# DJjjjhao/FIRA-ICSE

Measured on AMD Instinct MI355X. Metric: training commits/sec (FIRA default config), higher is better.
Workload: dtype f32; 1 GPU; BASELINE configs[1]: FIRA training step (fwd+bwd+Adam, dropout 0.1/0.2), batch 32 commits/GPU, fp32, 650-node graphs (mean nnz 1066/graph), vocab 24650; global_batch=32, parallelism=dp1

## Files before the change

fira_icse_amd/csrc/engine.h:

```cpp
#pragma once
#include "common.h"
#include <string>
#include <vector>

namespace fira {

int gemm_f32(hipStream_t s, int tA, int tB, int M, int N, int K, const float* A, int lda, const float* B, int ldb,
             float* C, int ldc, const float* bias, int flags, int splitk);
int gemm_f32_ex(hipStream_t s, int tA, int tB, int M, int N, int K, const float* A, int lda, const float* B, int ldb,
                float* C, int ldc, const float* bias, int flags, int splitk, float* colsum,
                const int32_t* c_rows = nullptr, const float* relu_mask = nullptr);
int gemm_bf16_ex(hipStream_t s, int tA, int tB, int M, int N, int K, const float* A, int lda, const float* B, int ldb,
                 float* C, int ldc, const float* bias, int flags, int splitk, float* colsum,
                 const int32_t* c_rows = nullptr, const float* relu_mask = nullptr);
struct ShadowEntry { int64_t offset; int rows, cols, pitch_t; int64_t offset_t; };
constexpr int SHADOW_MAX = 64;
struct ShadowTable {
    int n = 0;
    int64_t wbt_elems = 0;
    int tile_start[SHADOW_MAX + 1] = {0};
    ShadowEntry e[SHADOW_MAX];
};
int weight_shadows(hipStream_t s, const ShadowTable& tab, const float* P, uint16_t* Wb, uint16_t* WbT);
int gemm_bf16_wb_ex(hipStream_t s, int M, int N, int K, const float* A, int lda, const uint16_t* Bb, int ldb, float* C,
                    int ldc, const float* bias, int flags, int splitk, const int32_t* c_rows = nullptr,
                    const float* relu_mask = nullptr);
bool gemm_bf16_takes(int M, int N, int K);
struct GroupProblem {
    const float* A;
    const float* B;
    float* C;
    float* colsum;
    int M, N, K, lda, ldb, ldc, tiles_m, tiles_n, splitk, k_chunk;
};
constexpr int GROUP_MAX = 40;
struct GroupTable {
    int n = 0, chunk = 0;
    int wg_start[GROUP_MAX + 1] = {0};
    GroupProblem p[GROUP_MAX];
    void cost(double& flop, double& bytes) const {
        flop = bytes = 0;
        for (int i = 0; i < n; ++i) {
            const double M = p[i].M, N = p[i].N, K = p[i].K;
            flop += 2.0 * M * N * K;
            bytes += 4.0 * (M * K + N * K + M * N);
        }
    }
};
int gemm_group_plan(GroupProblem& q, int max_split);
int gemm_group_launch(hipStream_t s, const GroupTable& t);
int gemm_bf16_group_plan(GroupProblem& q, int max_split);
int gemm_bf16_group_launch(hipStream_t s, GroupTable& t);
struct PanelProblem {
    const float *A, *B;
    float *C, *colsum;
    float* part;
    int M, N, K, lda, ldb, ldc;
    int tiles_m, tiles_n, slabs, k_slab;
};
constexpr int PANEL_MAX = 48;
struct PanelTable {
    int n = 0;
    int wg_start[PANEL_MAX + 1] = {0};
    PanelProblem p[PANEL_MAX];
};
bool gemm_wgrad_panel_takes(int M, int N, int K, const float* A, int lda, const float* B, int ldb, int ldc);
int gemm_wgrad_panel_launch(hipStream_t s, int np, PanelTable& t, float* scratch, size_t scratch_floats);
struct WgradQueue {
    GroupTable tiled;
    PanelTable panels;
    float* scratch = nullptr;
    size_t scratch_floats = 0;
    int dtype = 0;
    void reset(int dtype_, float* scratch_, size_t floats) {
        tiled.n = 0; panels.n = 0;
        dtype = dtype_; scratch = scratch_; scratch_floats = scratch_ ? floats : 0;
    }
    bool full() const { return tiled.n == GROUP_MAX || panels.n == PANEL_MAX; }
    int panel_pending() const { return panels.n; }
    int add_tiled(int M, int N, int K, const float* A, int lda, const float* B, int ldb, float* C, int ldc, float* colsum,
                  int max_split = 0) {
        if (M <= 0 || N <= 0 || K <= 0) return 0;
        FIRA_REQUIRE(tiled.n < GROUP_MAX, "wgrad queue: tiled group full (fork and flush first)");
        GroupProblem& q = tiled.p[tiled.n];
        q.A = A; q.B = B; q.C = C; q.colsum = colsum;
        q.M = M; q.N = N; q.K = K; q.lda = lda; q.ldb = ldb; q.ldc = ldc;
        q.tiles_m = cdiv(M, 64); q.tiles_n = cdiv(N, 64);
        if (int rc = dtype == 1 ? gemm_bf16_group_plan(q, max_split) : gemm_group_plan(q, max_split)) return rc;
        tiled.wg_start[tiled.n + 1] = tiled.wg_start[tiled.n] + q.tiles_m * q.tiles_n * q.splitk;
        ++tiled.n;
        return 0;
    }
    int add_panel(int M, int N, int K, const float* A, int lda, const float* B, int ldb, float* C, int ldc, float* colsum) {
        FIRA_REQUIRE(panels.n < PANEL_MAX, "wgrad queue: panel table full (fork and flush first)");
        PanelProblem& q = panels.p[panels.n++];
        q.A = A; q.B = B; q.C = C; q.colsum = colsum;
        q.M = M; q.N = N; q.K = K; q.lda = lda; q.ldb = ldb; q.ldc = ldc;
        q.tiles_m = cdiv(M, 256); q.tiles_n = N / 256;
        q.slabs = 1; q.k_slab = K; q.part = nullptr;
        return 0;
    }
    int flush(hipStream_t s) {
        int rc = 0;
        if (tiled.n > 0) rc = dtype == 1 ? gemm_bf16_group_launch(s, tiled) : gemm_group_launch(s, tiled);
        tiled.n = 0;
        return rc ? rc : flush_panels(s);
    }
    int flush_panels(hipStream_t s) {
        const int rc = gemm_wgrad_panel_launch(s, dtype == 1 ? 1 : 3, panels, scratch, scratch_floats);
        panels.n = 0;
        return rc;
    }
};
constexpr int GEMM_SIDE_PAD = 1 << 8;
struct EpiRes;
bool gemm_tile32_takes(int tB, int M, int N, int K, const float* A, int lda, const float* B, int ldb);
bool gemm_tile32_try(hipStream_t s, int tB, int M, int N, int K, const float* A, int lda, const float* B, int ldb,
                     float* C, int ldc, const float* bias, int flags, int* rc, const int32_t* c_rows,
                     const float* relu_mask, const int32_t* a_rows, const EpiRes* er);
bool gemm_tile32_ln_try(hipStream_t s, int M, int N, const float* S, int lds, const float* W, const float* bias, float* Y,
                        int ldy, int flags, const float* gamma, const float* beta, float* x_out, float* stats_out, int* rc);
int gemm_tile32_lnb_blocks(int M);
bool gemm_tile32_lnb_try(hipStream_t s, int M, int N, const float* dy, const float* W, int ldw, float* dX, int lddx,
                         const float* relu_mask, const float* sum, const float* stats, const float* gamma, float* ds,
                         float* dx_drop, float* part, float dropout, uint64_t seed, uint32_t site, int* rc,
                         uint32_t idx0 = 0);
bool gemm_small_try(hipStream_t s, int tA, int tB, int M, int N, int K, const float* A, int lda, const float* B, int ldb,
                    float* C, int ldc, const float* bias, int flags, int* rc, const int32_t* c_rows = nullptr,
                    const float* relu_mask = nullptr);
int csr_spmm(hipStream_t s, int n_rows, const int32_t* rowptr, const int32_t* col, const float* val, const float* X,
             int ldx, float* Y, int ldy, int graph_rows, int variant);
int csr_spmm_ex(hipStream_t s, int n_rows, const int32_t* rowptr, const int32_t* col, const float* val, const float* X,
                int ldx, float* Y, int ldy, int graph_rows, int variant, int accum, float* rowsum);
int gcn_fused_fwd(hipStream_t s, int n_rows, const int32_t* rowptr, const int32_t* col, const float* val, const float* X,
                  const float* Wk, const float* bias, const float* r1_col, const float* gamma, const float* beta, float* sum,
                  float* y, float* stats, float* rowsum_out, const int32_t* slot2, float* y2, float dropout, uint64_t seed,
                  uint32_t site, int bf16, const uint16_t* Wx = nullptr);
int gcn_fused_bwd(hipStream_t s, int n_rows, const int32_t* rowptr, const int32_t* col, const float* val, const float* dY,
                  const float* Wk, float* u_out, float* acc_out, int bf16, const uint16_t* Wx = nullptr);
int gcn_split_planes(hipStream_t s, int n, const float* const* src, uint16_t* const* dst);
size_t head_logits_x3_scratch_elems(int R);
int head_logits_x3(hipStream_t s, int R, int V, const float* x, int ldx, const float* W, const float* bias, float* out, int ldo,
                   uint16_t* xplanes);
int transpose256(hipStream_t s, int nl, const float* W, float* Wt);
int linear_x3(hipStream_t s, int M, const float* X, int ldx, const uint16_t* Wx, int nb, const float* bias, float* out, int ldo,
              bool one_plane);
int split_planes_t(hipStream_t s, const float* W, int V, uint16_t* planes, bool one_plane);
int dgrad_x3_splitk(hipStream_t s, int M, int K, const float* A, int lda, const uint16_t* Wx, float* out, int ldo, bool one_plane);
int linear_x3_kacc(hipStream_t s, int M, const float* A, int lda, const uint16_t* Wx, int nkb, float* out, int ldo, bool accum,
                   bool one_plane);
int comb_fused_fwd(hipStream_t s, int n_rows, const float* Xc, const float* WqT, const float* WkT, const float* WoT,
                   const float* bqk, const float* bo, const float* vtab, int ldv, const int32_t* mark, float* qk, float* c,
                   const float* gamma, const float* beta, float* sum, float* y, const int32_t* y_rows, float* stats,
                   float dropout, uint64_t seed, uint32_t site_gate, uint32_t site_out, int bf16, const uint16_t* Wx = nullptr);
int comb_fused_bwd_parts();
int comb_fused_bwd(hipStream_t s, int n_rows, float* dG, const int32_t* rows, const float* sum, const float* stats,
                   const float* gamma, const float* Wo, const float* Wqk, const float* qk, const float* vtab, int ldv,
                   const int32_t* mark, float* dYc, float* dqk, float* part_ln, float* part_v, float dropout, uint64_t seed,
                   uint32_t site_gate, uint32_t site_out, int bf16, const uint16_t* WTx = nullptr);
struct TransposeTable { int n = 0; const float* src[24]; float* dst[24]; };
int transpose256_table(hipStream_t s, const TransposeTable& tab);
int embed_gather_fwd(hipStream_t s, int B, int L, const int32_t* idx, const float* table, const float* pos, float* out,
                     int out_bstride, int out_off);
int embed_grouped_bwd(hipStream_t s, int n_items, const int32_t* item_tok, const int32_t* item_ptr, const int32_t* rows,
                      float* dtable, const float* dnode);
int embed_list_bwd_small(hipStream_t s, int n, const int32_t* rows, const int32_t* ids, float* dtable, const float* dnode,
                         int table_rows);
int embed_gather_bwd(hipStream_t s, int B, int L, const int32_t* idx, float* dtable, const float* dout,
                     int out_bstride, int out_off, int padding_idx);
int embed_gather_bwd_small(hipStream_t s, int B, int L, const int32_t* idx, float* dtable, const float* dout,
                           int out_bstride, int out_off, int padding_idx, int table_rows);
int combination_fwd(hipStream_t s, int M, const float* qk, const float* vtab, int ldv, const int32_t* mark, float* out,
                    float dropout, uint64_t seed, uint32_t site);
int combination_bwd(hipStream_t s, int M, const float* qk, const float* vtab, int ldv, const int32_t* mark,
                    const float* dout, float* dqk, float* dvtab, int lddv, float dropout, uint64_t seed, uint32_t site,
                    float* part = nullptr);
int combination_bwd_blocks(int M);
struct RedEntry { float* dst; const float* src; int width, n_part, stride; };
constexpr int RED_MAX = 96;
struct RedTable {
    int n = 0;
    int wg_start[RED_MAX + 1] = {0};
    RedEntry e[RED_MAX];
};
int deferred_reduce(hipStream_t s, RedTable& tab);
int add_layernorm_fwd(hipStream_t s, int M, float* x, const float* res, const float* gamma, const float* beta,
                      float* y, float* stats, float dropout, uint64_t seed, uint32_t site, const int32_t* y_rows, const float* r1_row = nullptr,
                      const float* r1_col = nullptr,
                      const int32_t* slot2 = nullptr, float* y2 = nullptr,
                      uint32_t idx0 = 0);
bool gemm_bf16_k256_try(hipStream_t s, int M, int N, int K, const float* A, int lda, const uint16_t* Bb, int ldb, float* C,
                        int ldc, const float* bias, int flags, const int32_t* c_rows, const float* relu_mask, int* rc);
// ... 185 lines not shown
```

fira_icse_amd/csrc/engine.hip:

```cpp
#include "engine.h"
#include <hip/hip_ext.h>
#include "epilogue.h"
#include "decode_row.h"
#include <stdlib.h>
#include <map>
#include <mutex>

namespace fira {

static int64_t shadow_wbt_elems(const Layout& L);

struct Arena {
    char* base;
    size_t used = 0;
    explicit Arena(void* b) : base((char*)b) {}
    template <typename T>
    T* get(size_t n) {
        size_t bytes = (n * sizeof(T) + 255) / 256 * 256;
        T* p = base ? (T*)(base + used) : nullptr;
        used += bytes;
        return p;
    }
    float* f(size_t n) { return get<float>(n); }
};
// ... 540 lines not shown
    hipEvent_t ev_shadow = nullptr;
    struct Lane { hipStream_t s; int b0, nb, r0, nr; } lanes[2] = {};
    Call call;
};
typedef Ctx::Lane Lane;

static int adam_sched_check(const fira_adam_opts* adam) { return adam && adam->sched ? fira_lr_schedule_check(adam->sched) : 0; }

static AdamRowsTables adam_rows_tables(const Layout& L, float* params, const fira_adam_opts& ad, int32_t* row_step) {
    AdamRowsTables tb;
    tb.p = params; tb.m = ad.m; tb.v = ad.v;
    tb.off[0] = L.dec_emb; tb.off[1] = L.emb;
    tb.rows[0] = tb.rows[1] = L.d.vocab;
    tb.last = row_step;
    return tb;
}

static int decoder_lanes(Ctx& c) {
    constexpr int DEC_LANES_MIN_ROWS = 768;
    static const int forced = [] { const char* e = getenv("FIRA_DEC_LANES"); return e ? (atoi(e) >= 2 ? 2 : 1) : 0; }();
    const int want = forced ? forced : (c.Td >= DEC_LANES_MIN_ROWS ? 2 : 1);
    c.call.lanes = 1;
    c.lanes[0] = Lane{c.s, 0, c.pl->B, 0, c.Td};
    const fira_batch& bt = *c.bt;
    if (want < 2 || !c.dec_off || !bt.dec_off_host || bt.B < 2 || !side_on() || c.serial || !c.kv_ragged) return 0;
    SideStream& sd = side();
    if (!sd.lane) {
        if (hipStreamCreateWithFlags(&sd.lane, hipStreamNonBlocking) != hipSuccess) return set_err("lane stream: create failed");
    }
    int bm = 1, best = 1 << 30;
    for (int b = 1; b < bt.B; ++b) {
        const int d = abs(2 * bt.dec_off_host[b] - c.Td);
        if (d < best) { best = d; bm = b; }
    }
    const int rm = bt.dec_off_host[bm];
    if (rm <= 0 || rm >= c.Td || bt.dec_off_host[bt.B] != c.Td) return 0;
    c.call.lanes = 2;
    c.lanes[0] = Lane{c.s, 0, bm, 0, rm};
    c.lanes[1] = Lane{sd.lane, bm, bt.B - bm, rm, c.Td - rm};
    return 0;
}
static int lanes_fork(Ctx& c) {
    for (int k = 1; k < c.call.lanes; ++k) {
        hipEvent_t e = side().ev();
        if (hipEventRecord(e, c.s) != hipSuccess || hipStreamWaitEvent(c.lanes[k].s, e, 0) != hipSuccess) return set_err("lane fork failed");
    }
    return 0;
}
static int lanes_join(Ctx& c) {
    for (int k = 1; k < c.call.lanes; ++k) {
        hipEvent_t e = side().ev();
        if (hipEventRecord(e, c.lanes[k].s) != hipSuccess || hipStreamWaitEvent(c.s, e, 0) != hipSuccess) return set_err("lane join failed");
    }
    return 0;
}
static int lanes_fork_to(Ctx& c, hipStream_t target) {
    for (int k = 0; k < c.call.lanes; ++k) {
        hipEvent_t e = side().ev();
        if (hipEventRecord(e, k ? c.lanes[k].s : c.s) != hipSuccess || hipStreamWaitEvent(target, e, 0) != hipSuccess) return set_err("lane -> side stream fork failed");
    }
    return 0;
}

enum { PANEL_ENC = 1, PANEL_DEC = 2, PANEL_VOCAB = 4, PANEL_KV = 8 };
static inline bool panel_takes(const Call& call, int cls, int M, int N, int K, const float* dY, int lddy, const float* X, int ldx) {
    const int mask = call.dtype == 1 ? 13 : 15;
    return (mask & cls) && gemm_wgrad_panel_takes(N, K, M, dY, lddy, X, ldx, K);
}

static inline int wgrad_on(Call& call, hipStream_t ws, int panel_cls, int M, int N, int K, const float* dY, int lddy,
                           const float* X, int ldx, float* dW, float* db) {
    if (call.wq.panel_pending() == 0 && panel_takes(call, panel_cls, M, N, K, dY, lddy, X, ldx)) {
        TRY(call.wq.add_panel(N, K, M, dY, lddy, X, ldx, dW, K, db));
        return call.wq.flush_panels(ws);
    }
    return gemm_any(call, ws, 1, 0, N, K, M, dY, lddy, X, ldx, dW, K, nullptr, FIRA_GEMM_ACCUM | side_pad(ws), 0, db);
}
static inline int linear_wgrad(Ctx& c, int M, int N, int K, const float* dY, int lddy, const float* X, int ldx, float* dW,
                               float* db, int panel_cls = 0) {
    if (side_on()) TRY(side_fork(c.s));
    return wgrad_on(c.call, wgrad_stream(c.s), panel_cls, M, N, K, dY, lddy, X, ldx, dW, db);
}

static inline int flush_wgrads(Ctx& c) {
    if (!side_on()) return 0;
    TRY(lanes_fork_to(c, side().stream));
    return c.call.wq.flush(side().stream);
}
static inline int wgrad_queued(Ctx& c, bool grouping, int queue_cls, int direct_cls, int max_split, int M, int N, int K,
                               const float* dY, int lddy, const float* X, int ldx, float* dW, float* db) {
    Call& call = c.call;
    if (!grouping) return linear_wgrad(c, M, N, K, dY, lddy, X, ldx, dW, db, direct_cls);
    if (call.wq.full()) TRY(flush_wgrads(c));
    if (panel_takes(call, queue_cls, M, N, K, dY, lddy, X, ldx)) return call.wq.add_panel(N, K, M, dY, lddy, X, ldx, dW, K, db);
    if (call.dtype == 1 && !gemm_bf16_takes(N, K, M)) return linear_wgrad(c, M, N, K, dY, lddy, X, ldx, dW, db);
    return call.wq.add_tiled(N, K, M, dY, lddy, X, ldx, dW, K, db, max_split);
}
static inline int linear_wgrad_grouped(Ctx& c, int M, int N, int K, const float* dY, int lddy, const float* X, int ldx,
                                       float* dW, float* db, int max_split = 0) {
    return wgrad_queued(c, side_on(), PANEL_DEC, 0, max_split, M, N, K, dY, lddy, X, ldx, dW, db);
}
static inline bool enc_group_on() {
    static const bool off = [] { const char* e = getenv("FIRA_ENC_WGRAD_GROUP"); return e && e[0] == '0'; }();
    return !off && side_on();
}
static inline int enc_wgrad(Ctx& c, int M, int N, int K, const float* dY, int lddy, const float* X, int ldx, float* dW, float* db) {
    return wgrad_queued(c, enc_group_on(), PANEL_ENC, PANEL_ENC, 32, M, N, K, dY, lddy, X, ldx, dW, db);
}

static inline bool fold_one_launch(int nl) { return nl <= 10; }
static inline bool comb_x3_on(int nl) { return nl <= 8; }
static inline bool gcn_x3_on(const Call& call, int nl) { return call.gcn_fused() && fold_one_launch(nl); }
static inline bool kv_x3_on(int nl) { return nl * 2 <= 24; }

static AdamRowsView lazy_view(const Ctx& c, int table) {
    const AdamVals& lz = c.step.lazy;
    if (!lz.rows) return AdamRowsView();
    return adam_rows_view(adam_rows_tables(*c.L, nullptr, lz.ad, lz.rows), table, lz.lr, lz.ad.beta1, lz.ad.beta2, lz.ad.eps, lz.ad.step - 1);
}
static int adam_rows_prefetch(Ctx& c, hipStream_t st) {
    const fira_batch& bt = *c.bt;
    const Plan& p = *c.pl;
    const fira_adam_opts& ad = c.step.lazy.ad;
    AdamRowsLists ls{};
    auto add = [&](const int32_t* ids, int n, int table) {
        if (!ids || n <= 0) return;
        const int k = ls.n_lists++;
        ls.ids[k] = ids; ls.table[k] = table;
        ls.end[k] = (k ? ls.end[k - 1] : 0) + n;
    };
    add(bt.tar, p.B * p.T, 0);
    return adam_rows_catchup(st, adam_rows_tables(*c.L, const_cast<float*>(c.P), ad, c.step.lazy.rows), &ls, c.step.lazy.lr, ad.beta1, ad.beta2, ad.eps,
                             ad.step - 1);
}

static int encoder_forward(Ctx& c, bool defer_memory_proj) {
    Plan& p = *c.pl;
    const Layout& L = *c.L;
    const fira_batch& bt = *c.bt;
    hipStream_t s = c.s;
    const int D = FIRA_D, Nc = bt.n_nodes, Cc = bt.n_code, Mc = bt.n_mem, KV = p.nl * 2 * D;
    hipEvent_t ev_fold0 = nullptr, ev_fold = nullptr, ev_comb = nullptr;
    bool fold_waited = false;
    {
        const bool ax = side_on() && !c.serial;
        hipStream_t fs = ax ? side().aux : s;
        if (ax) TRY(aux_fork(s));
        TransposeTable tt;
        for (int l = 0; l < p.nl && tt.n + 3 <= 24; ++l) {
            const EncLayer& w = L.enc[l];
            float* dst = p.WcT + (size_t)l * 3 * D * D;
            tt.src[tt.n] = c.P + w.wqk; tt.dst[tt.n++] = dst;
            tt.src[tt.n] = c.P + w.wqk + (size_t)D * D; tt.dst[tt.n++] = dst + (size_t)D * D;
            tt.src[tt.n] = c.P + w.wo; tt.dst[tt.n++] = dst + (size_t)2 * D * D;
        }
        TRY(transpose256_table(fs, tt));
        if (comb_x3_on(p.nl)) {
            const float* src[48];
            uint16_t* dst[48];
            int n = 0;
            for (int l = 0; l < p.nl; ++l) {
                const EncLayer& w = L.enc[l];
                const float* st[3] = {c.P + w.wqk, c.P + w.wqk + (size_t)D * D, c.P + w.wo};
                for (int j = 0; j < 3; ++j) {
                    src[n] = st[j]; dst[n++] = p.WcX + ((size_t)l * 3 + j) * 3 * D * D;
                    if (c.G) { src[n] = p.WcT + ((size_t)l * 3 + j) * D * D; dst[n++] = p.WcTX + ((size_t)l * 3 + j) * 3 * D * D; }
                }
            }
            TRY(gcn_split_planes(fs, n, src, dst));
        }
// ... 171 lines not shown
                    float* sum = const_cast<float*>(st.pend_sum) + r0 * D;
                    const bool fused = gemm_tile32_ln_try(s, nr, N, sum, D, W, b, Y + r0 * N, N, flags, st.pend_g, st.pend_b,
                                                          st.pend_y + r0 * D, st.pend_st + r0 * 2, &rc);
                    if (!fused)
                        rc = add_layernorm_fwd(s, nr, sum, nullptr, st.pend_g, st.pend_b, st.pend_y + r0 * D, st.pend_st + r0 * 2, 0.f, 0, 0,
                                               nullptr);
                    st.pend_sum = nullptr;
                    if (rc || fused) return rc;
                }
                return linear(c.call, s, nr, N, D, st.x + r0 * D, D, W, b, Y + r0 * N, N, flags);
            };
            auto close_block = [&](int K, const float* X, const float* W, const float* b, const float* res, const float* g,
                                   const float* be, float* sum, float* y, float* stt, uint32_t site_id, bool may_defer,
                                   const int32_t* slot2, float* y2, int n2, const int32_t* rows2) -> int {
                int rc = 0;
                if (may_defer && linear_presum(c.call, s, nr, K, X + r0 * K, K, W, b, res + r0 * D, sum + r0 * D, c.p_drop, c.seed, site_id,
                                               &rc, idx0)) {
                    st.pend_sum = sum; st.pend_g = g; st.pend_b = be; st.pend_y = y; st.pend_st = stt;
                    return rc;
                }
                return linear_ln(c.call, s, nr, K, X + r0 * K, K, W, b, res + r0 * D, g, be, sum + r0 * D, y + r0 * D, stt + r0 * 2, c.p_drop,
                                 c.seed, site_id, nullptr, nullptr, nullptr, slot2 ? slot2 + r0 : nullptr, y2, n2, rows2, idx0);
            };
            const int32_t* q_off = c.dec_off ? c.dec_off + ln.b0 : nullptr;
            TRY(consume(3 * D, c.P + w.wqkv, c.P + w.bqkv, e.qkv, 0));
            TRY(attention_fwd(s, ln.nb, H, p.T, p.T, e.qkv, 3 * D, e.qkv + D, 3 * D, e.qkv + 2 * D, 3 * D, p.tar_valid + (size_t)ln.b0 * p.T,
                              1, 0, e.ao, D, q_off, 1, attn_bf16(c.call)));
            TRY(close_block(D, e.ao, c.P + w.wo_s, c.P + w.bo_s, st.x, c.P + w.lns_g, c.P + w.lns_b, e.s_a, e.x_a, e.st_a,
                            site(l, SITE_SELF), true, nullptr, nullptr, 0, nullptr));
            st.x = e.x_a;
            TRY(consume(D, c.P + w.wq_c, c.P + w.bq_c, e.qc, 0));
            if (c.deferred) {
                int m = l;
                while (m < p.nl - 1 && c.ev_kv[m] == nullptr) ++m;
                if (c.ev_kv[m] != nullptr && st.kv_waited < m + 1) {
                    TRY(main_wait(s, c.ev_kv[m], __LINE__));
                    st.kv_waited = m + 1;
                }
            }
            TRY(attention_fwd(s, ln.nb, H, p.T, Sm, e.qc, D, p.kv_all + l * 2 * D, p.kvp, p.kv_all + l * 2 * D + D, p.kvp,
                              c.kv_ragged ? p.mem_valid_c : p.mem_valid, 0, 0, e.ao2, D, q_off, 0, attn_bf16(c.call),
                              c.kv_ragged ? p.mem_off + ln.b0 : nullptr));
            TRY(close_block(D, e.ao2, c.P + w.wo_c, c.P + w.bo_c, e.x_a, c.P + w.lnc_g, c.P + w.lnc_b, e.s_c, e.x_c, e.st_c,
                            site(l, SITE_CROSS), true, nullptr, nullptr, 0, nullptr));
            st.x = e.x_c;
            TRY(consume(p.F, c.P + w.w1, c.P + w.b1, e.h, FIRA_GEMM_RELU));
            const bool head_copy = last && c.rows != nullptr && c.R > 0;
            TRY(close_block(p.F, e.h, c.P + w.w2, c.P + w.b2, e.x_c, c.P + w.lnf_g, c.P + w.lnf_b, e.s_f, e.x_f, e.st_f,
                            site(l, SITE_FFN), !last, head_copy ? p.compact_row : nullptr, head_copy ? p.dec_c : nullptr,
                            head_copy ? c.R : 0, head_copy ? c.rows : nullptr));
            st.x = e.x_f;
        }
    }
    TRY(lanes_join(c));
    return 0;
}

static int head_forward(Ctx& c, int R, const int32_t* rows, float* loss_sum, int32_t* n_tok, int32_t* argmax_out,
                        int want_grad) {
    Plan& p = *c.pl;
    const Layout& L = *c.L;
    hipStream_t s = c.s;
    const int D = FIRA_D, Sm = p.L + p.S;
    const float* dec = p.dec[p.nl - 1].x_f;
    const float* dec_rows = (c.rows != nullptr && rows == c.rows) ? p.dec_c : dec;
    if (dec_rows == dec && R != c.Td) {
        TRY(rows_gather_idx(s, R, p.dec_c, dec, rows));
        dec_rows = p.dec_c;
    }
    if (c.call.dtype == 0 && R >= 64 && R <= p.TB)
        TRY(head_logits_x3(s, R, p.V, dec_rows, D, c.P + L.wout, c.P + L.bout, p.logits, p.ldl, p.xh_planes));
    else
    TRY(linear(c.call, s, R, p.V, D, dec_rows, D, c.P + L.wout, c.P + L.bout, p.logits, p.ldl));
    TRY(gemm_any(c.call, s, 0, 1, c.Td, D, D, dec, D, c.P + L.wt, D, p.tgt, D, nullptr, 0, 0, nullptr));
    if (c.deferred) TRY(main_wait(s, c.ev_src, __LINE__));
    TRY(copy_score_fwd_ex(s, p.B, p.T, Sm, p.src, p.tgt, c.P + L.wres, c.P + L.bres, p.score, 1, p.mem_valid,
                          argmax_out ? nullptr : c.bt->tar_label, p.V, c.dec_off));
    TRY(linear(c.call, s, c.Td, 2, D, dec, D, c.P + L.wp, c.P + L.bp, p.gate, 2));
    TRY(head_loss(s, c.Td, p.T, p.V, Sm, p.compact_row, p.logits, p.ldl, p.score, p.mem_valid, p.gate,
                  c.bt->tar_label, loss_sum, n_tok, argmax_out, want_grad, c.row_bt));
    return 0;
}

static inline int enc_wgrad_every(int n_rows, int n_layers) {
    static const int forced = [] { const char* e = getenv("FIRA_ENC_WGRAD_EVERY"); const int v = e ? atoi(e) : 0; return v >= 1 ? v : 0; }();
    if (forced) return forced;
    return n_rows <= 32768 ? std::max(1, n_layers) : 1;
}

static int group_a_final_stream(hipStream_t s, hipStream_t* out) {
    SideStream& sd = side();
    *out = s;
    if (side_on()) {
        TRY(aux_fork(s));
        hipEvent_t e2 = sd.ev();
        if (hipEventRecord(e2, sd.stream) != hipSuccess || hipStreamWaitEvent(sd.aux, e2, 0) != hipSuccess)
            return set_err("group-A mark: weight-gradient stream mark failed");
        *out = sd.aux;
    }
    return 0;
}

struct BwdMid {
    hipEvent_t ev_dmem = nullptr;
    hipEvent_t ev_groupA = nullptr;
};

static int backward_decoder(Ctx& c, int R, const int32_t* rows, BwdMid& mid) {
    Plan& p = *c.pl;
    const Step& st = c.step;
    const Layout& L = *c.L;
    hipStream_t s = c.s;
    const int D = FIRA_D, H = L.d.n_head, KV = p.nl * 2 * D, Sm = p.L + p.S;
    const fira_batch& bt = *c.bt;
    const int Nc = bt.n_nodes, Cc = bt.n_code, Mc = bt.n_mem;
    const float* dec = p.dec[p.nl - 1].x_f;
    float* G = c.G;

    c.call.wq.reset(c.call.dtype, p.panel_scratch, p.panel_floats);
    c.call.red.reset(p.red_buf, p.red_cap);
    const bool so = side_on();
    hipStream_t ss = aux_stream(s);
    hipEvent_t ev_dfc = nullptr;
    if (c.ev_zero) TRY(main_wait(s, c.ev_zero, __LINE__));
    else TRY(zero(s, p.zero_beg, (size_t)((char*)p.zero_end - (char*)p.zero_beg)));
    if (R > 0) {
        if (so) TRY(aux_fork(s));
        if (c.wout_planes) TRY(dgrad_x3_splitk(ss, R, p.V, p.logits, p.ldl, p.WoutTX, p.ddec_c, D, c.call.dtype == 1));
        else
        TRY(gemm_any(c.call, ss, 0, 0, R, D, p.V, p.logits, p.ldl, c.P + L.wout, D, p.ddec_c, D, nullptr, FIRA_GEMM_ACCUM, 0,
                        nullptr));
        if (so) TRY(side_mark(&ev_dfc));
    }
    if (R > 0)
        TRY(linear_wgrad(c, R, p.V, D, p.logits, p.ldl, (c.rows != nullptr && rows == c.rows) ? p.dec_c : dec, D, G + L.wout,
                         G + L.bout, PANEL_VOCAB));
    if (c.call.dtype == 0) TRY(rank2_rows(s, c.Td, p.gate, c.P + L.wp, p.ddec));
    else TRY(linear_dgrad(c.call, s, c.Td, 2, D, p.gate, 2, c.P + L.wp, p.ddec, D, false));
    TRY(linear_wgrad_grouped(c, c.Td, 2, D, p.gate, 2, dec, D, G + L.wp, G + L.bp));
    {
        const int nb = copy_score_bwd_blocks(p.B, Sm);
        float* part = c.call.red.alloc((size_t)nb * COPY_PART_STRIDE);
        TRY(copy_score_bwd_ex(s, p.B, p.T, Sm, p.src, p.tgt, c.P + L.wres, p.score, p.dsrc, p.dtgt, G + L.wres, G + L.bres,
                              p.mem_valid, part, c.dec_off));
        if (part) {
            c.call.red.add(G + L.wres, part, D, nb, COPY_PART_STRIDE);
            c.call.red.add(G + L.bres, part + D, 1, nb, COPY_PART_STRIDE);
        }
    }
    TRY(linear_dgrad(c.call, s, c.Td, D, D, p.dtgt, D, c.P + L.wt, p.ddec, D, true));
    TRY(linear_wgrad_grouped(c, c.Td, D, D, p.dtgt, D, dec, D, G + L.wt, nullptr));
    TRY(rows_move(s, 0, Mc, D, p.dsrc_c, p.dsrc, bt.mem_dst, nullptr));
    if (so) TRY(aux_fork(s));
    TRY(linear_dgrad(c.call, ss, Mc, D, D, p.dsrc_c, D, c.P + L.ws, p.dmem_c, D, false));
    TRY(linear_wgrad_grouped(c, Mc, D, D, p.dsrc_c, D, p.mem_c, D, G + L.ws, nullptr, 8));
    if (R > 0) {
        if (ev_dfc) TRY(main_wait(s, ev_dfc, __LINE__));
        TRY(rows_scatter_add_idx(s, R, p.ddec_c, p.ddec, rows));
    }

    float *bx = p.ddec, *by = p.dT_a, *bz = p.dT_c;
    constexpr int DEC_WGRAD_EVERY = 3;
    const int dec_every = p.nl % DEC_WGRAD_EVERY != 0 ? 0 : DEC_WGRAD_EVERY;
    {
    ProfScope prof_region(s, PROF_DEC_REGION, 0.0);
    TRY(lanes_fork(c));
    auto aux_fork_all = [&]() -> int { return c.call.lanes > 1 ? lanes_fork_to(c, side().aux) : aux_fork(s); };
    for (int l = p.nl - 1; l >= 0; --l) {
        ProfDecoderTag prof_tag;
        const DecLayer& w = L.dec[l];
// ... 180 lines not shown
    float* dXn = p.dXa;
    float* other = p.dXb;
    UnfoldTable unfold_tab;
    static const bool unfold_late_off = [] { const char* e = getenv("FIRA_UNFOLD_LATE"); return e && e[0] == '0'; }();
    const bool unfold_late = !unfold_late_off && enc_group_on() && p.nl <= 16;
    const int wgrad_every = unfold_late ? enc_wgrad_every(Nc, p.nl) : 1;
    const float *uf_dW21[16], *uf_W1[16], *uf_W2[16];
    float *uf_dW1[16], *uf_dW2[16];
    int uf_n = 0;
    if (!c.ev_zero) TRY(zero(s, dXn, (size_t)Nc * D * sizeof(float)));
    if (ev_dmem) TRY(main_wait(s, ev_dmem, __LINE__));
    TRY(rows_move(s, 1, Mc, D, dXn, p.dmem_c, nullptr, bt.mem_rows));
    for (int l = p.nl - 1; l >= 0; --l) {
        const EncLayer& w = L.enc[l];
        EncSave& e = p.enc[l];
        EncGrad& g = p.encg[l];
        float* dc21 = p.dc21 + (size_t)l * D;
        bool sums = false;
        const bool room = unfold_tab.n < 16;
        TRY(ln_bwd(c.call, s, Nc, dXn, e.s2, e.st2, c.P + w.ln2g, other, g.dY2, G + w.ln2g, G + w.ln2b, c.p_gcn,
                              c.seed, site(l, SITE_GCN), nullptr, room ? p.rsum : nullptr, G + w.fc2b, dc21, &sums));
        if (sums) unfold_tab.e[unfold_tab.n++] = UnfoldEntry{c.P + w.fc2w, c.P + w.fc1b, dc21, G + w.fc2w, G + w.fc1b};
        float* dW21 = p.dW21 + (size_t)l * D * D;
        const bool grouped = enc_group_on();
        bool flushed = false;
        auto unfold = [&]() -> int {
            hipStream_t ws = wgrad_stream(s);
            if (ws != s && (!grouped || (!flushed && (!sums || !unfold_late)))) TRY(side_fork(s));
            if (!sums) TRY(colsum(ws, Nc, D, g.dY2, D, dc21, p.rsum));
            if (unfold_late) {
                uf_dW21[uf_n] = dW21; uf_W1[uf_n] = c.P + w.fc1w; uf_W2[uf_n] = c.P + w.fc2w;
                uf_dW1[uf_n] = G + w.fc1w; uf_dW2[uf_n] = G + w.fc2w;
                ++uf_n;
            } else {
            TRY(gemm_f32_ex(ws, 0, 1, D, D, D, dW21, D, c.P + w.fc1w, D, G + w.fc2w, D, nullptr, FIRA_GEMM_ACCUM | side_pad(ws), 0, nullptr));
            TRY(gemm_f32_ex(ws, 1, 0, D, D, D, c.P + w.fc2w, D, dW21, D, G + w.fc1w, D, nullptr, FIRA_GEMM_ACCUM | side_pad(ws), 0, nullptr));
            }
            if (!sums) TRY(gcn_bias_unfold(ws, c.P + w.fc2w, c.P + w.fc1b, dc21, G + w.fc2w, G + w.fc1b));
            return 0;
        };
        if (c.call.gcn_fused()) {
            TRY(gcn_fused_bwd(s, Nc, bt.rowptr, bt.col, bt.val, g.dY2, p.W21 + (size_t)l * D * D, e.Z, other, c.call.dtype == 1,
                              gcn_x3_on(c.call, p.nl) ? p.W21tx + (size_t)l * 3 * D * D : nullptr));
            TRY(enc_wgrad(c, Nc, D, D, e.Z, D, p.X[l], D, dW21, nullptr));
            if (!sums) TRY(colsum(s, Nc, D, g.dY2, D, G + w.fc2b));
            if (!grouped) TRY(unfold());
        } else {
        TRY(enc_wgrad(c, Nc, D, D, g.dY2, D, e.Z, D, dW21, sums ? nullptr : G + w.fc2b));
        if (!grouped) TRY(unfold());
        TRY(linear_dgrad(c.call, s, Nc, D, D, g.dY2, D, p.W21 + (size_t)l * D * D, p.dNB2, D, false));
        TRY(csr_spmm_ex(s, Nc, bt.rowptr, bt.col, bt.val, p.dNB2, D, other, D, 0, 1, 1, nullptr));
        }
        const int nb_comb = comb_fused_bwd_parts();
        float* part_ln = c.call.red.alloc((size_t)nb_comb * 6 * D, 6);
        const bool comb_done = part_ln != nullptr;
        if (comb_done) {
            float* part_v = part_ln + (size_t)nb_comb * 2 * D;
            TRY(comb_fused_bwd(s, Cc, other, bt.code_rows, e.s1, e.st1, c.P + w.ln1g, c.P + w.wo, c.P + w.wqk, e.qk,
                               p.vtab_all + l * D, p.nl * D, bt.code_mark, g.dYc, g.dqk, part_ln, part_v, c.p_drop, c.seed,
                               site(l, SITE_GATE), site(l, SITE_COMB_OUT), c.call.dtype == 1,
                               comb_x3_on(p.nl) ? p.WcTX + (size_t)l * 9 * D * D : nullptr));
            c.call.red.add(G + w.ln1g, part_ln, D, nb_comb, 2 * D);
            c.call.red.add(G + w.ln1b, part_ln + D, D, nb_comb, 2 * D);
            for (int k = 0; k < 4; ++k)
                c.call.red.add(p.dvtab_all + (size_t)k * p.nl * D + l * D, part_v + k * D, D, nb_comb, 4 * D);
            TRY(enc_wgrad(c, Cc, D, D, g.dYc, D, e.c, D, G + w.wo, G + w.bo));
        } else {
        TRY(ln_bwd(c.call, s, Cc, other, e.s1, e.st1, c.P + w.ln1g, other, g.dYc, G + w.ln1g, G + w.ln1b, c.p_drop,
                              c.seed, site(l, SITE_COMB_OUT), bt.code_rows));
        TRY(enc_wgrad(c, Cc, D, D, g.dYc, D, e.c, D, G + w.wo, G + w.bo));
        TRY(linear_dgrad(c.call, s, Cc, D, D, g.dYc, D, c.P + w.wo, p.dCB_a, D, false));
        {
            const int nb = combination_bwd_blocks(Cc);
            float* part = c.call.red.alloc((size_t)nb * 4 * D);
            TRY(combination_bwd(s, Cc, e.qk, p.vtab_all + l * D, p.nl * D, bt.code_mark, p.dCB_a, g.dqk,
                                p.dvtab_all + l * D, p.nl * D, c.p_drop, c.seed, site(l, SITE_GATE), part));
            if (part)
                for (int k = 0; k < 4; ++k)
                    c.call.red.add(p.dvtab_all + (size_t)k * p.nl * D + l * D, part + k * D, D, nb, 4 * D);
        }
        }
        TRY(enc_wgrad(c, Cc, 2 * D, D, g.dqk, 2 * D, e.Xc, D, G + w.wqk, G + w.bqk));
        if (grouped) {
            if ((p.nl - l) % wgrad_every == 0 || l == 0) { TRY(flush_wgrads(c)); flushed = true; }
            TRY(unfold());
        }
        if (!comb_done)
            TRY(gemm_any(c.call, s, 0, 0, Cc, D, 2 * D, g.dqk, 2 * D, c.P + w.wqk, D, other, D, nullptr, FIRA_GEMM_ACCUM, 0, nullptr,
                         bt.code_rows));
        float* tmp = dXn; dXn = other; other = tmp;
    }
    if (uf_n > 0) TRY(gcn_unfold_products(side().stream, uf_n, uf_dW21, uf_W1, uf_W2, uf_dW1, uf_dW2));
    hipEvent_t ev_tail = nullptr;
    int64_t adam_b0 = L.split;
    {
        const bool ax = side_on();
        hipStream_t rs = aux_stream(s);
        if (ax) TRY(aux_fork(s));
        TRY(deferred_reduce(rs, c.call.red.tab));
        TRY(gemm_f32_ex(rs, 1, 0, p.nl * D, D, 4, p.dvtab_all, p.nl * D, c.P + L.mark_emb, D, G + L.w2_all, D, nullptr,
                        FIRA_GEMM_ACCUM, 1, G + L.b2_all));
        TRY(gemm_f32_ex(rs, 0, 0, 3, D, p.nl * D, p.dvtab_all + (size_t)p.nl * D, p.nl * D, c.P + L.w2_all, D, G + L.mark_emb + D, D,
                        nullptr, FIRA_GEMM_ACCUM, std::max(2, p.nl), nullptr));
        if (ax) TRY(side_mark(&ev_tail));
    }
    if (bt.emb_item_tok && bt.emb_item_ptr && bt.emb_rows && bt.ast_rows && bt.ast_ids && L.d.ast_vocab <= 128) {
        TRY(embed_grouped_bwd(s, bt.n_emb_items, bt.emb_item_tok, bt.emb_item_ptr, bt.emb_rows, G + L.emb, dXn));
        TRY(embed_list_bwd_small(s, bt.n_ast_items, bt.ast_rows, bt.ast_ids, G + L.ast_emb, dXn, L.d.ast_vocab));
    } else {
        TRY(zero(s, p.H, (size_t)p.NB * D * sizeof(float)));
        TRY(rows_move(s, 1, Nc, D, p.H, dXn, nullptr, bt.node_rows));
        TRY(embed_gather_bwd(s, p.B, p.L, bt.sou, G + L.emb, p.H, p.N, 0, 0));
        TRY(embed_gather_bwd(s, p.B, p.S, bt.sub_token, G + L.emb, p.H, p.N, p.L, 0));
        if (L.d.ast_vocab <= 128)
            TRY(embed_gather_bwd_small(s, p.B, p.A, bt.ast_change, G + L.ast_emb, p.H, p.N, p.L + p.S, 0, L.d.ast_vocab));
        else
            TRY(embed_gather_bwd(s, p.B, p.A, bt.ast_change, G + L.ast_emb, p.H, p.N, p.L + p.S, 0));
    }
    TRY(update_early(c, ev_groupA, &adam_b0));
    if (ev_tail) TRY(main_wait(s, ev_tail, __LINE__));
    if (side_on()) TRY(side_join(s, __LINE__));
    TRY(gcn_bias_unfold_all(s, unfold_tab));
    return update_close(c, adam_b0);
}

static int check_batch(const fira_batch* b) {
    FIRA_REQUIRE(b && b->B > 0, "empty batch");
    FIRA_REQUIRE(b->sou && b->mark && b->ast_change && b->sub_token && b->rowptr && b->col && b->val,
                 "batch has null encoder inputs");
    FIRA_REQUIRE(b->node_rows && b->code_rows && b->code_mark && b->mem_rows && b->mem_dst,
                 "batch has null node lists (node_rows / code_rows / code_mark / mem_rows / mem_dst)");
    FIRA_REQUIRE(b->n_nodes > 0 && b->n_code > 0 && b->n_mem > 0 && b->n_code <= b->n_nodes && b->n_mem <= b->n_nodes,
                 "inconsistent node counts %d / %d / %d", b->n_nodes, b->n_code, b->n_mem);
    return 0;
}
static int check_counts(const fira_batch* b, const Plan& p) {
    FIRA_REQUIRE(b->n_nodes <= p.NB && b->n_code <= p.CB && b->n_mem <= p.MB, "node lists exceed the batch geometry");
    return 0;
}

struct DecodePlan {
    Plan enc;
    int BR;
    float *kc[2], *vc[2];
    int32_t* hist[2];
    float *x, *q, *qkv, *ao, *s, *xa, *qc, *xc, *h, *tgt, *score, *gate, *logits;
    float* wsT;
    uint16_t* kv16;
    size_t build(void* ws, const fira_dims& d, int B, int n_beam, int flags = 0) {
        size_t used = enc.build(ws, d, B, false);
        Arena a(ws ? (char*)ws + used : nullptr);
        BR = B * n_beam;
        const size_t D = FIRA_D, T = d.tar_len, cache = (size_t)d.n_layer * BR * T * D;
        for (int i = 0; i < 2; ++i) {
            kc[i] = a.f(cache); vc[i] = a.f(cache);
            hist[i] = a.get<int32_t>((size_t)BR * T);
        }
        x = a.f(BR * D); q = a.f(BR * D); qkv = a.f(BR * 3 * D); ao = a.f(BR * D); s = a.f(BR * D); xa = a.f(BR * D); qc = a.f(BR * D);
        xc = a.f(BR * D); h = a.f((size_t)BR * d.d_ff); tgt = a.f(BR * D);
        score = a.f((size_t)BR * (d.sou_len + d.sub_len)); gate = a.f((size_t)BR * 2);
        logits = a.f((size_t)BR * enc.ldl);
        wsT = a.f((size_t)d.n_layer * 2 * D * D);
        kv16 = (flags & FIRA_DECODE_KV_BF16) ? a.get<uint16_t>((size_t)enc.MB * enc.kvp) : nullptr;
        return used + a.used;
    }
};

// ... 619 lines not shown
```

fira_icse_amd/csrc/gemm_wgrad_panel.hip:

```cpp
#include "engine.h"
#include "epilogue.h"
#include <algorithm>
#include <stdlib.h>

namespace fira {

typedef __bf16 pbf16x8 __attribute__((ext_vector_type(8)));
typedef __bf16 pbf16x2 __attribute__((ext_vector_type(2)));
typedef float pf32x2 __attribute__((ext_vector_type(2)));
typedef float pf32x16 __attribute__((ext_vector_type(16)));

constexpr int PN_T = 256;
constexpr int PN_KB = 16;
constexpr int PN_PART = PN_T * 32;

__device__ __forceinline__ int pn_unit(int row, int kh) { return kh * PN_T + row; }

__device__ __forceinline__ uint32_t pn_pack(float a, float b) {
    pf32x2 v = {a, b};
    return __builtin_bit_cast(uint32_t, __builtin_convertvector(v, pbf16x2));
}
__device__ __forceinline__ void pn_rest(float& a, float& b, uint32_t pk) {
    a -= __builtin_bit_cast(float, pk << 16);
    b -= __builtin_bit_cast(float, pk & 0xffff0000u);
// ... 119 lines not shown
        for (int i = t; i < PN_T; i += 512) pn_cs[i] = 0.f;
        __syncthreads();
        if (opnd == 0) { atomicAdd(&pn_cs[2 * cb], cs0); atomicAdd(&pn_cs[2 * cb + 1], cs1); }
        __syncthreads();
        for (int i = t; i < PN_T; i += 512)
            if (m0 + i < q.M) unsafeAtomicAdd(&q.colsum[m0 + i], pn_cs[i]);
    }
    if (q.slabs > 1) {
        float* pt = q.part + ((size_t)(tm * q.tiles_n + tn) * q.slabs + z) * (PN_T * PN_T);
#pragma unroll
        for (int j = 0; j < 2; ++j)
#pragma unroll
            for (int i = 0; i < 4; ++i)
#pragma unroll
                for (int r = 0; r < 16; ++r)
                    pt[(wm * 128 + i * 32 + (r & 3) + 8 * (r >> 2) + 4 * kh) * PN_T + wn * 64 + j * 32 + l31] = acc[i][j][r];
        return;
    }
    const rsrc_t rC = buf_rsrc(q.C, 0x7fffffffu);
#pragma unroll
    for (int j = 0; j < 2; ++j) {
        const int col = n0 + wn * 64 + j * 32 + l31;
#pragma unroll
        for (int i = 0; i < 4; ++i) {
            unsigned off[16];
            float old[16];
#pragma unroll
            for (int r = 0; r < 16; ++r) {
                const int row = m0 + wm * 128 + i * 32 + (r & 3) + 8 * (r >> 2) + 4 * kh;
                off[r] = (row < q.M && col < q.N) ? ((unsigned)row * (unsigned)q.ldc + (unsigned)col) * 4u : FIRA_OOB;
                old[r] = buf_load_f32(rC, off[r]);
            }
#pragma unroll
            for (int r = 0; r < 16; ++r)
                __builtin_amdgcn_raw_buffer_store_b32(__builtin_bit_cast(unsigned, old[r] + acc[i][j][r]), rC, off[r], 0, 0);
        }
    }
}

__global__ __launch_bounds__(256) void wgrad_panel_reduce_kernel(const PanelTable tab) {
    int b = blockIdx.x, pi = 0;
    for (pi = 0; pi < tab.n; ++pi) {
        const PanelProblem& q = tab.p[pi];
        if (q.slabs <= 1) continue;
        const int nb = q.tiles_m * q.tiles_n * 64;
        if (b < nb) break;
        b -= nb;
    }
    if (pi >= tab.n) return;
    const PanelProblem& q = tab.p[pi];
    const int tile = b >> 6, idx = (b & 63) * 256 + threadIdx.x;
    const int tm = tile / q.tiles_n, tn = tile % q.tiles_n;
    const int row = tm * PN_T + (idx >> 6), col = tn * PN_T + (idx & 63) * 4;
    const float4* pt = reinterpret_cast<const float4*>(q.part + (size_t)tile * q.slabs * (PN_T * PN_T)) + idx;
    float4 a = make_float4(0.f, 0.f, 0.f, 0.f);
    int z = 0;
    for (; z + 4 <= q.slabs; z += 4) {
        const float4 x0 = pt[(size_t)z * (PN_T * PN_T / 4)], x1 = pt[(size_t)(z + 1) * (PN_T * PN_T / 4)];
        const float4 x2 = pt[(size_t)(z + 2) * (PN_T * PN_T / 4)], x3 = pt[(size_t)(z + 3) * (PN_T * PN_T / 4)];
        a.x += (x0.x + x1.x) + (x2.x + x3.x); a.y += (x0.y + x1.y) + (x2.y + x3.y);
        a.z += (x0.z + x1.z) + (x2.z + x3.z); a.w += (x0.w + x1.w) + (x2.w + x3.w);
    }
    for (; z < q.slabs; ++z) {
        const float4 x = pt[(size_t)z * (PN_T * PN_T / 4)];
        a.x += x.x; a.y += x.y; a.z += x.z; a.w += x.w;
    }
    if (row >= q.M || col >= q.N) return;
    float4* c = reinterpret_cast<float4*>(q.C + (size_t)row * q.ldc + col);
    if ((((uintptr_t)c) & 15) == 0) {
        float4 o = *c;
        o.x += a.x; o.y += a.y; o.z += a.z; o.w += a.w;
        *c = o;
    } else {
        float* cf = reinterpret_cast<float*>(c);
        cf[0] += a.x; cf[1] += a.y; cf[2] += a.z; cf[3] += a.w;
    }
}

bool gemm_wgrad_panel_takes(int M, int N, int K, const float* A, int lda, const float* B, int ldb, int ldc) {
    return M >= 32 && N >= PN_T && N % PN_T == 0 && K >= 1 && lda % 2 == 0 && ldb % 2 == 0 &&
           ((uintptr_t)A % 8) == 0 && ((uintptr_t)B % 8) == 0 && (long)K * lda * 4 < 0x7fffffffL && (long)K * ldb * 4 < 0x7fffffffL &&
           epilogue_fits(M, ldc);
}
int gemm_wgrad_panel_launch(hipStream_t s, int np, PanelTable& t, float* scratch, size_t scratch_floats) {
    if (t.n == 0) return 0;
    constexpr int target_wgs = 256;
    double work = 0, flop = 0, bytes = 0;
    for (int i = 0; i < t.n; ++i) {
        const PanelProblem& q = t.p[i];
        work += (double)q.tiles_m * q.tiles_n * q.K;
        flop += 2.0 * q.M * q.N * (double)q.K;
        bytes += 4.0 * ((double)q.M * q.K + (double)q.N * q.K + (double)q.M * q.N);
    }
    int tiles_total = 0;
    for (int i = 0; i < t.n; ++i) tiles_total += t.p[i].tiles_m * t.p[i].tiles_n;
    int per = std::max(256, (int)((work / target_wgs + PN_KB - 1) / PN_KB) * PN_KB);
    if (3 * tiles_total >= target_wgs) per = 1 << 30;
    size_t need = 0;
    for (int pass = 0; pass < 8; ++pass) {
        need = 0;
        for (int i = 0; i < t.n; ++i) {
            PanelProblem& q = t.p[i];
            q.slabs = scratch ? std::max(1, cdiv(q.K, per)) : 1;
            q.k_slab = cdiv(cdiv(q.K, q.slabs), PN_KB) * PN_KB;
            q.slabs = cdiv(q.K, q.k_slab);
            if (q.slabs > 1) need += (size_t)q.tiles_m * q.tiles_n * q.slabs * (PN_T * PN_T);
        }
        if (need <= scratch_floats) break;
        per *= 2;
    }
    if (need > scratch_floats) {
        for (int i = 0; i < t.n; ++i) { t.p[i].slabs = 1; t.p[i].k_slab = cdiv(t.p[i].K, PN_KB) * PN_KB; }
        need = 0;
    }
    size_t off = 0;
    int bands = 0;
    for (int i = 0; i < t.n; ++i) {
        PanelProblem& q = t.p[i];
        q.part = nullptr;
        if (q.slabs > 1) {
            q.part = scratch + off;
            off += (size_t)q.tiles_m * q.tiles_n * q.slabs * (PN_T * PN_T);
            bands += q.tiles_m * q.tiles_n * 64;
        }
        t.wg_start[i + 1] = t.wg_start[i] + q.tiles_m * q.tiles_n * q.slabs;
    }
    ProfScope prof(s, PROF_GEMM, flop, bytes);
    const size_t lds = (size_t)2 * 2 * np * PN_PART;
    if (np == 3) {
        if (int rc = raise_dynamic_lds<wgrad_panel_kernel<3>>(lds, "wgrad_panel")) return rc;
        hipLaunchKernelGGL(wgrad_panel_kernel<3>, dim3(t.wg_start[t.n]), dim3(512), lds, s, t);
    } else {
        if (int rc = raise_dynamic_lds<wgrad_panel_kernel<1>>(lds, "wgrad_panel")) return rc;
        hipLaunchKernelGGL(wgrad_panel_kernel<1>, dim3(t.wg_start[t.n]), dim3(512), lds, s, t);
    }
    if (bands > 0) hipLaunchKernelGGL(wgrad_panel_reduce_kernel, dim3(bands), dim3(256), 0, s, t);
    FIRA_CHECK_LAUNCH("wgrad_panel");
    return 0;
}
}

extern "C" int fira_gemm_wgrad_panel(void* stream, int dtype, int M, int N, int K, const float* A, int lda, const float* B, int ldb,
                                     float* C, int ldc, float* colsum, float* scratch, size_t scratch_floats) {
    FIRA_REQUIRE(A && B && C && (dtype == 0 || dtype == 1), "fira_gemm_wgrad_panel: bad argument");
    FIRA_REQUIRE(fira::gemm_wgrad_panel_takes(M, N, K, A, lda, B, ldb, ldc),
                 "fira_gemm_wgrad_panel: shape %d x %d x %d / alignment not taken (M >= 32, N %% 256 == 0, even pitches)", M, N, K);
    fira::WgradQueue q;
    q.reset(dtype, scratch, scratch_floats);
    if (int rc = q.add_panel(M, N, K, A, lda, B, ldb, C, ldc, colsum)) return rc;
    return q.flush((hipStream_t)stream);
}
```

Before: 13780 commits/s.

## Flush encoder wgrads in two batches with a narrower early panel launch

In the small-row encoder backward, queued weight-gradient GEMMs are now flushed in two batches instead of once at the end: after layer 1 and again at layer 0. The layer-1 flush targets half as many workgroups for the split-K panel kernel, so that batch runs on the side stream while layer 0's data-gradient work continues. This is meant to overlap wgrad compute with the remaining critical-path work and shorten the tail. The cost is an extra launch and flush, plus possible contention between the side-stream wgrads and the main-stream work.

```diff
diff --git a/fira_icse_amd/csrc/engine.h b/fira_icse_amd/csrc/engine.h
--- a/fira_icse_amd/csrc/engine.h
+++ b/fira_icse_amd/csrc/engine.h
@@ -65,7 +65,8 @@
     PanelProblem p[PANEL_MAX];
 };
 bool gemm_wgrad_panel_takes(int M, int N, int K, const float* A, int lda, const float* B, int ldb, int ldc);
-int gemm_wgrad_panel_launch(hipStream_t s, int np, PanelTable& t, float* scratch, size_t scratch_floats);
+constexpr int PANEL_WGS_ALL = 256;
+int gemm_wgrad_panel_launch(hipStream_t s, int np, PanelTable& t, float* scratch, size_t scratch_floats, int target_wgs = PANEL_WGS_ALL);
 struct WgradQueue {
     GroupTable tiled;
     PanelTable panels;
@@ -100,14 +101,14 @@
         q.slabs = 1; q.k_slab = K; q.part = nullptr;
         return 0;
     }
-    int flush(hipStream_t s) {
+    int flush(hipStream_t s, int panel_wgs = PANEL_WGS_ALL) {
         int rc = 0;
         if (tiled.n > 0) rc = dtype == 1 ? gemm_bf16_group_launch(s, tiled) : gemm_group_launch(s, tiled);
         tiled.n = 0;
-        return rc ? rc : flush_panels(s);
-    }
-    int flush_panels(hipStream_t s) {
-        const int rc = gemm_wgrad_panel_launch(s, dtype == 1 ? 1 : 3, panels, scratch, scratch_floats);
+        return rc ? rc : flush_panels(s, panel_wgs);
+    }
+    int flush_panels(hipStream_t s, int panel_wgs = PANEL_WGS_ALL) {
+        const int rc = gemm_wgrad_panel_launch(s, dtype == 1 ? 1 : 3, panels, scratch, scratch_floats, panel_wgs);
         panels.n = 0;
         return rc;
     }
diff --git a/fira_icse_amd/csrc/engine.hip b/fira_icse_amd/csrc/engine.hip
--- a/fira_icse_amd/csrc/engine.hip
+++ b/fira_icse_amd/csrc/engine.hip
@@ -646,10 +646,10 @@
     return wgrad_on(c.call, wgrad_stream(c.s), panel_cls, M, N, K, dY, lddy, X, ldx, dW, db);
 }
 
-static inline int flush_wgrads(Ctx& c) {
+static inline int flush_wgrads(Ctx& c, int panel_wgs = PANEL_WGS_ALL) {
     if (!side_on()) return 0;
     TRY(lanes_fork_to(c, side().stream));
-    return c.call.wq.flush(side().stream);
+    return c.call.wq.flush(side().stream, panel_wgs);
 }
 static inline int wgrad_queued(Ctx& c, bool grouping, int queue_cls, int direct_cls, int max_split, int M, int N, int K,
                                const float* dY, int lddy, const float* X, int ldx, float* dW, float* db) {
@@ -987,10 +987,17 @@
     return 0;
 }
 
+constexpr int ENC_WGRAD_LAST_APART = -1;
+constexpr int ENC_WGRAD_EARLY_WGS = 128;
 static inline int enc_wgrad_every(int n_rows, int n_layers) {
-    static const int forced = [] { const char* e = getenv("FIRA_ENC_WGRAD_EVERY"); const int v = e ? atoi(e) : 0; return v >= 1 ? v : 0; }();
-    if (forced) return forced;
-    return n_rows <= 32768 ? std::max(1, n_layers) : 1;
+    static const int forced = [] {
+        const char* e = getenv("FIRA_ENC_WGRAD_EVERY");
+        const int v = e ? atoi(e) : 0;
+        return v >= 1 || v == ENC_WGRAD_LAST_APART ? v : 0;
+    }();
+    const int every = forced ? forced : n_rows <= 32768 ? ENC_WGRAD_LAST_APART : 1;
+    if (every == ENC_WGRAD_LAST_APART && n_layers < 2) return 1;
+    return every;
 }
 
 static int group_a_final_stream(hipStream_t s, hipStream_t* out) {
@@ -1337,7 +1344,9 @@
         }
         TRY(enc_wgrad(c, Cc, 2 * D, D, g.dqk, 2 * D, e.Xc, D, G + w.wqk, G + w.bqk));
         if (grouped) {
-            if ((p.nl - l) % wgrad_every == 0 || l == 0) { TRY(flush_wgrads(c)); flushed = true; }
+            const bool flush_now = wgrad_every == ENC_WGRAD_LAST_APART ? l <= 1 : ((p.nl - l) % wgrad_every == 0 || l == 0);
+            const bool early = wgrad_every == ENC_WGRAD_LAST_APART && l == 1;
+            if (flush_now) { TRY(flush_wgrads(c, early ? ENC_WGRAD_EARLY_WGS : PANEL_WGS_ALL)); flushed = true; }
             TRY(unfold());
         }
         if (!comb_done)
diff --git a/fira_icse_amd/csrc/gemm_wgrad_panel.hip b/fira_icse_amd/csrc/gemm_wgrad_panel.hip
--- a/fira_icse_amd/csrc/gemm_wgrad_panel.hip
+++ b/fira_icse_amd/csrc/gemm_wgrad_panel.hip
@@ -225,9 +225,9 @@
            ((uintptr_t)A % 8) == 0 && ((uintptr_t)B % 8) == 0 && (long)K * lda * 4 < 0x7fffffffL && (long)K * ldb * 4 < 0x7fffffffL &&
            epilogue_fits(M, ldc);
 }
-int gemm_wgrad_panel_launch(hipStream_t s, int np, PanelTable& t, float* scratch, size_t scratch_floats) {
+int gemm_wgrad_panel_launch(hipStream_t s, int np, PanelTable& t, float* scratch, size_t scratch_floats, int target_wgs) {
     if (t.n == 0) return 0;
-    constexpr int target_wgs = 256;
+    target_wgs = std::min(std::max(target_wgs, 8), PANEL_WGS_ALL);
     double work = 0, flop = 0, bytes = 0;
     for (int i = 0; i < t.n; ++i) {
         const PanelProblem& q = t.p[i];
@@ -238,7 +238,7 @@
     int tiles_total = 0;
     for (int i = 0; i < t.n; ++i) tiles_total += t.p[i].tiles_m * t.p[i].tiles_n;
     int per = std::max(256, (int)((work / target_wgs + PN_KB - 1) / PN_KB) * PN_KB);
-    if (3 * tiles_total >= target_wgs) per = 1 << 30;
+    if (3 * tiles_total >= PANEL_WGS_ALL) per = 1 << 30;
     size_t need = 0;
     for (int pass = 0; pass < 8; ++pass) {
         need = 0;
```

Result: no change. 13850 commits/s (median of 6 runs) (+0.5%).
